# AdrianPerezHerrero/HDP-GPC

Hardware: AMD Instinct MI355X
Metric: GP log-lik evals/sec (NxK batch, T-point segments) (higher is better)
Workload: dtype f64; 1 GPU; BASELINE configs[1]: synthetic 2048 segments x 8 clusters, T=128, fp64, irregular segment grids (per-pair Gram + Cholesky + score); segments=2048, segments_per_gpu=2048, clusters=8, T=128

## Files before the change

### hdpgpc_amd/csrc/hgp_internal.hpp

```cpp
#pragma once
#include <hip/hip_runtime.h>
#include <stddef.h>
#include <stdint.h>
#include <stdlib.h>

#include <type_traits>
#include <vector>

#include "../../include/hdpgpc_hip.h"

constexpr int WAVES = 4;

static inline int launch_status() {
  hipError_t e = hipGetLastError();
  return e == hipSuccess ? 0 : 1000 + (int)e;
}

static inline int nb_for(int n) {
  int nb = (n + 15) / 16;
  nb = (nb + 1) & ~1;
  return nb < 2 ? 2 : nb;
}

template <class F> static inline auto dispatch_nb_wave(int T, F&& f) {
  switch (nb_for(T)) {
    case 2: return f(std::integral_constant<int, 2>{});
    case 4: return f(std::integral_constant<int, 4>{});
    case 6: return f(std::integral_constant<int, 6>{});
    default: return f(std::integral_constant<int, 8>{});
  }
}
template <class F> static inline auto dispatch_nb_coop(int T, F&& f) {
  return T <= 192 ? f(std::integral_constant<int, 12>{}) : f(std::integral_constant<int, 16>{});
}
template <class F> static inline auto dispatch_nb(int NB, F&& f) {
  return NB <= 8 ? dispatch_nb_wave(16 * NB, f) : dispatch_nb_coop(16 * NB, f);
}
template <class F> static inline auto dispatch_bool(bool on, F&& f) {
  return on ? f(std::true_type{}) : f(std::false_type{});
}

static inline bool env_on(const char* name) {
  const char* v = getenv(name);
  return v && v[0] && v[0] != '0';
}

constexpr double PAIRS_CUT = 55.45177444479562;
constexpr int PAIRS_FB_CAP = 65536;

static inline int acc_grid_for(int nb) { return nb > 8 ? 256 : 512; }

struct hgp_pairs_plan {
  int T, K, TP, NB;
  std::vector<double> theta;
  std::vector<int32_t> perm;
  std::vector<int> grp_beg, grp_end;
  std::vector<double> grp_ell;
  double *d_theta, *d_scal, *d_A, *d_S, *d_Z, *d_Kinv, *d_P, *d_Q, *d_Mp, *d_ap, *d_xb;
  int32_t* d_perm;
  bool coop = false;
  double* d_escr = nullptr;
  int32_t* d_eflags = nullptr;
  int nscr = 0;
  long escr_stride = 0;
  double acc_tol = 1e-9;
  double* d_Lop = nullptr;
  double* d_LTop = nullptr;
  double* d_Dop = nullptr;
  double* d_Sop = nullptr;
  double* d_mu = nullptr;
  int32_t* d_acc_list = nullptr;
  double* d_sscr = nullptr;
  int32_t* d_fb = nullptr;
  int score_out = 0;
};

struct PlanReuse {
  long long* key_jit;
  int32_t* valid;
  int32_t* same;
  int32_t* factored;
  int32_t* info;
  static constexpr size_t BYTES_PER_CLUSTER = sizeof(long long) + 4 * sizeof(int32_t);
};
static inline PlanReuse plan_reuse(const hgp_pairs_plan* p) {
  long long* key = reinterpret_cast<long long*>(p->d_Q);
  int32_t* w = reinterpret_cast<int32_t*>(key + p->K);
  return PlanReuse{key, w, w + p->K, w + 2 * p->K, w + 3 * p->K};
}

struct PotrfArgs {
  double* A;
  int T, b;
  double jitter_rel, add;
  double* Linv;
  double* logdet;
  int32_t* info;
  double* Aout = nullptr;
  const int32_t* src_idx = nullptr;
};
int hgp_internal_potrf_ws(const double* A, const int32_t* idx, int T, int b, double jitter_rel, double* L, int32_t* info, hipStream_t st);
int hgp_internal_potrf_coop(const PotrfArgs& a, hipStream_t st);

struct InvArgs {
  const double* A;
  int T, b;
  double jitter_rel, add;
  double* Linv;
  int32_t* info;
  const double* rhs = nullptr;
  int rhs_trans = 0;
  int symmetric = 0;
  const int32_t* rhs_on = nullptr;
  double* rhs_out = nullptr;
  const int32_t* keep = nullptr;
};
static_assert(offsetof(InvArgs, rhs_on) == 64, "InvArgs: the plain forms' arguments fill the first 64 bytes");
int hgp_internal_chol_inverse(const InvArgs& a, int NB, double* factor_out, hipStream_t st);
void hgp_internal_wave_inverse(const InvArgs& a, hipStream_t st);
void hgp_internal_trtri(const double* L, double* Z, int T, int b, const int32_t* info, hipStream_t st);
int hgp_internal_ensure_dynamic_lds(const void* fn, size_t bytes);

struct GemmArgs {
  const double* A;
  const double* B;
  double* C;
  int M, N, Kd, lda, ldb, ldc;
  long sA, sB, sC;
  double alpha, beta;
  int tA, tB;
  int nb2 = 1;
  long sA2 = 0, sB2 = 0, sC2 = 0;
  const double* D = nullptr;
  int ldd = 0;
  long sD = 0;
  int boff = 0;
  int triA = 0;
};
int hgp_internal_gemm(const GemmArgs& a, int batch, hipStream_t st);
void hgp_internal_dot_batched(const double* X, const double* Y, long sX, long sY, long n, double scale, int accumulate, double* out, int b, hipStream_t st);
void hgp_internal_colnorm_diag(const double* Z, const double* S, long sS, int T, double scale, int accumulate, double* out, int b, hipStream_t st);
void hgp_internal_sub_batched(const double* A, const double* B, long sA, long sB, long n, double* C, int b, hipStream_t st);

int hgp_internal_acc_prep(hgp_pairs_plan* p, const double* mean, bool flags_done, hipStream_t st);
int hgp_internal_pairs_acc(const hgp_pairs_plan* p, const double* x, const double* y, int N, int Ts, const double* first_noise,
                           const int32_t* sel, double* out_quad, double* out_logdet, int32_t* out_info, hipStream_t st);
int hgp_internal_pairs_acc_ragged(const hgp_pairs_plan* p, const double* x, const double* y, int N, int ld, const int32_t* seg_len,
                                  const double* first_noise, const int32_t* sel, double* out_quad, double* out_logdet,
                                  int32_t* out_info, hipStream_t st);
size_t hgp_internal_acc_bytes(int TP, int K, size_t* sizes );

int hgp_internal_lat_coop(const double* f_cur, const double* f_prev, const double* A, const double* Gamma, const double* P, int T, int b,
                          double* out, int32_t* info, double* ws, hipStream_t st);
int hgp_internal_mniw_coop(const double* M, const double* Sigma, const double* m_mean, const double* scale, long prior_stride, int T, int b,
                           double* out, int32_t* info, double* ws, hipStream_t st);

struct PairsArgs {
  const double* x;
  const double* y;
  int N, Ts;
  const double* xb;
  int T;
  const double* Mp;
  const double* ap;
  const double* scal;
  const int32_t* perm;
  int kbeg, kend;
  double ell;
  const double* first_noise;
  const int32_t* sel;
#ifdef HGP_STAMPS
  unsigned long long* stamps;
#endif
  int K;
  double* out_quad;
  double* out_logdet;
  int32_t* out_info;
  double* escr;
  int32_t* eflags;
  int nscr;
  long escr_stride;
  int flags;
  double score_add;
  int score_on;
  int32_t* fb;
};

struct PairsRagArgs : PairsArgs {
  const int32_t* seg_len;
};
template <class Args> constexpr bool pairs_ragged = std::is_base_of<PairsRagArgs, Args>::value;

struct PairsSegArgs : PairsArgs {
  const double* store;
};

#ifdef HGP_STAMPS
extern unsigned long long* hgp_internal_stamp_dev;
#endif
int hgp_internal_pairs_fast(const PairsArgs& a, int NB, bool coop, hipStream_t st);
int hgp_internal_pairs_fast_ragged(const PairsRagArgs& a, int NB, bool coop, hipStream_t st);
int hgp_internal_pairs_listed(const PairsArgs& a, int NB, hipStream_t st);
int hgp_internal_pairs_listed_ragged(const PairsRagArgs& a, int NB, hipStream_t st);
```

### hdpgpc_amd/csrc/hgp_pairs_acc.hip

```cpp
#include <hip/hip_runtime.h>
#include <math.h>
#include <stdint.h>

#include "hgp_internal.hpp"
#include "tile_f64.hpp"

using namespace hgp;

namespace {

__host__ __device__ constexpr int ntl(int NB) { return NB * (NB - 1) / 2; }
__host__ __device__ constexpr int tl(int K, int Kp) { return K * (K - 1) / 2 + Kp; }

#ifndef HGP_PAIRS_RAGGED_TU
__global__ void k_acc_flags(double* scal, int K, double tol, int32_t* acc_list) {
  if (threadIdx.x != 0 || blockIdx.x != 0) return;
  int n = 0;
  for (int k = 0; k < K; ++k) {
    const double ck = scal[8 * k] * scal[8 * k + 6];
    const double bound = F64_EPS * ck * ck;
    const bool flag = (tol == 0.0) || (tol > 0.0 && !(bound <= tol));
    scal[8 * k + 7] = flag ? 1.0 : 0.0;
    if (flag) acc_list[1 + n++] = k;
  }
  acc_list[0] = n;
}

template <int NB>
__global__ __launch_bounds__(64) void k_acc_factor(double* A, int TP, const double* scal, int32_t* info, int32_t* factored) {
  __shared__ __attribute__((aligned(16))) double scr[DIAG_SCR];
  const int k = blockIdx.x, lane = threadIdx.x;
  if (scal[8 * k + 7] == 0.0) return;
  if (factored[k] != 0) return;
  double* Ak = A + (size_t)k * TP * TP;
  d4 U[NB * (NB + 1) / 2];
  d4 R[NB];
  load_upper_only<NB>(U, Ak, TP, TP, lane);
  PivotAcc pa;
  pa.init();
  wave_factor<NB, 0>(U, R, scr, nullptr, nullptr, lane, pa, Ak, TP, TP);
  if (lane == 0 && info && pa.info != 0) info[k] = pa.info;
  if (lane == 0) factored[k] = 1;
}

struct AccPrepArgs {
  const double* L;
  const double* S;
  const double* mean;
  const double* scal;
  int T, TP, NB;
  double* Lop;
  double* LTop;
  double* Dop;
  double* Sop;
  double* mu;
};

__global__ __launch_bounds__(256) void k_acc_prep(AccPrepArgs a) {
  const int k = blockIdx.x;
  if (a.scal[8 * k + 7] == 0.0) return;
  const int lane = threadIdx.x & 63, g = lane >> 4, c = lane & 15;
  const int wv = blockIdx.y * 4 + (threadIdx.x >> 6), nwv = gridDim.y * 4;
  const int NB = a.NB, TP = a.TP;
  const double* L = a.L + (size_t)k * TP * TP;
  const double* S = a.S + (size_t)k * TP * TP;
  const int nl = ntl(NB);
  double* Lop = a.Lop + (size_t)k * nl * 256;
  double* LTop = a.LTop + (size_t)k * nl * 256;
  double* Dop = a.Dop + (size_t)k * 4 * NB * 256;
  double* Sop = a.Sop + (size_t)k * NB * NB * 256;
  if (blockIdx.y == 0)
    for (int i = threadIdx.x; i < TP; i += 256) a.mu[(size_t)k * TP + i] = (i < a.T) ? a.mean[(size_t)k * a.T + i] : 0.0;
  const int items = nl + NB + NB * NB;
  for (int it = wv; it < items; it += nwv) {
    if (it < nl) {
      int Kb = 1;
      while (tl(Kb + 1, 0) <= it) ++Kb;
      const int Kp = it - tl(Kb, 0);
      d4 lo, lt;
#pragma unroll
      for (int s = 0; s < 4; ++s) {
        lo[s] = L[(size_t)(16 * Kb + c) * TP + 16 * Kp + 4 * s + g];
        lt[s] = L[(size_t)(16 * Kb + 4 * s + g) * TP + 16 * Kp + c];
      }
      *reinterpret_cast<d4*>(Lop + ((size_t)it * 64 + lane) * 4) = lo;
      *reinterpret_cast<d4*>(LTop + ((size_t)it * 64 + lane) * 4) = lt;
    } else if (it < nl + NB) {
      const int Kb = it - nl;
      const double* D = L + (size_t)(16 * Kb) * TP + 16 * Kb;
      d4 a1, a2, a1t, a2t;
#pragma unroll
      for (int r = 0; r < 4; ++r) {
        const double* B = D + (size_t)(4 * r) * TP + 4 * r;
        const double l00 = B[0], l10 = B[TP], l11 = B[TP + 1], l20 = B[2 * TP], l21 = B[2 * TP + 1], l22 = B[2 * TP + 2],
                     l30 = B[3 * (size_t)TP], l31 = B[3 * (size_t)TP + 1], l32 = B[3 * (size_t)TP + 2], l33 = B[3 * (size_t)TP + 3];
        double w[4][4];
#pragma unroll
        for (int i = 0; i < 4; ++i)
#pragma unroll
          for (int j = 0; j < 4; ++j) w[i][j] = 0.0;
        const double r0 = 1.0 / l00, r1 = 1.0 / l11, r2 = 1.0 / l22, r3 = 1.0 / l33;
        w[0][0] = r0;
        w[1][0] = -(l10 * w[0][0]) * r1;
        w[2][0] = -(l20 * w[0][0] + l21 * w[1][0]) * r2;
        w[3][0] = -(l30 * w[0][0] + l31 * w[1][0] + l32 * w[2][0]) * r3;
        w[1][1] = r1;
        w[2][1] = -(l21 * w[1][1]) * r2;
        w[3][1] = -(l31 * w[1][1] + l32 * w[2][1]) * r3;
        w[2][2] = r2;
        w[3][2] = -(l32 * w[2][2]) * r3;
        w[3][3] = r3;
        const int ci = c & 3;
        double wf = 0.0, wt = 0.0;
#pragma unroll
        for (int i = 0; i < 4; ++i)
#pragma unroll
          for (int j = 0; j < 4; ++j) {
            if (i == ci && j == g) wf = w[i][j];
            if (i == g && j == ci) wt = w[i][j];
          }
        const bool mine = (c >> 2) == r;
        a1[r] = mine ? wf : 0.0;
        a1t[r] = mine ? wt : 0.0;
        a2[r] = (c >= 4 * r + 4) ? D[(size_t)c * TP + 4 * r + g] : 0.0;
        a2t[r] = (c < 4 * r) ? D[(size_t)(4 * r + g) * TP + c] : 0.0;
      }
      *reinterpret_cast<d4*>(Dop + ((size_t)(0 * NB + Kb) * 64 + lane) * 4) = a1;
      *reinterpret_cast<d4*>(Dop + ((size_t)(1 * NB + Kb) * 64 + lane) * 4) = a2;
      *reinterpret_cast<d4*>(Dop + ((size_t)(2 * NB + Kb) * 64 + lane) * 4) = a1t;
      *reinterpret_cast<d4*>(Dop + ((size_t)(3 * NB + Kb) * 64 + lane) * 4) = a2t;
    } else {
      const int t = it - nl - NB, Kb = t / NB, Kp = t % NB;
      d4 so;
#pragma unroll
      for (int s = 0; s < 4; ++s) so[s] = S[(size_t)(16 * Kp + 4 * s + g) * TP + 16 * Kb + c];
      *reinterpret_cast<d4*>(Sop + ((size_t)t * 64 + lane) * 4) = so;
    }
  }
}

#endif

struct AccArgs {
  const double* x;
  const double* y;
  int N, Ts;
  const double* xb;
  int T;
  const double* scal;
  const double* mu;
  const double* Lop;
  const double* LTop;
  const double* Dop;
  const double* Sop;
  const int32_t* acc_list;
  const double* first_noise;
  const int32_t* sel;
  int K;
  double* out_quad;
  double* out_logdet;
  int32_t* out_info;
  double* sscr;
  double score_add;
  int score_on;
};
struct AccRagArgs : AccArgs {
  const int32_t* seg_len;
};
template <class Args> constexpr bool acc_ragged = std::is_base_of<AccRagArgs, Args>::value;
#ifdef HGP_PAIRS_RAGGED_TU
using KArgs = AccRagArgs;
#define ACC_SEG_LEN(a, n, ld) __builtin_amdgcn_readfirstlane((a).seg_len[n])
#define ACC_SCORE_ADD(a, Ts) (-0.5 * (double)(Ts) * 1.8378770664093453)
#else
using KArgs = AccArgs;
#define ACC_SEG_LEN(a, n, ld) (ld)
#define ACC_SCORE_ADD(a, Ts) (a).score_add
#endif

template <int NB>
struct PairsAccLds {
  static constexpr int TP = 16 * NB;
  static constexpr int ROWBUF = 0, WBUF = ROWBUF + NB * 256, DVEC = WBUF + 256, XS = DVEC + TP, YS = XS + TP, XBS = YS + TP,
                       MUS = XBS + TP, SCR = MUS + TP, RED = SCR + DIAG_SCR, REDI = RED + 32;
  static constexpr size_t BYTES = sizeof(double) * REDI + sizeof(int) * 16;
  static_assert(WBUF % 2 == 0 && SCR % 2 == 0 && BYTES <= LDS_MAX_BYTES, "k_pairs_acc: LDS");
  HGP_LDS_DOUBLES(rowbuf, ROWBUF)
  HGP_LDS_DOUBLES(Wbuf, WBUF)
  HGP_LDS_DOUBLES(dvec, DVEC)
  HGP_LDS_DOUBLES(xs, XS)
  HGP_LDS_DOUBLES(ys, YS)
  HGP_LDS_DOUBLES(xbs, XBS)
  HGP_LDS_DOUBLES(mus, MUS)
  HGP_LDS_DOUBLES(scr, SCR)
  HGP_LDS_DOUBLES(red, RED)
  HGP_LDS_INTS(redi, REDI, 0)
};

__device__ __forceinline__ d4 ld4(const double* base, unsigned off) { return *reinterpret_cast<const d4*>(base + off); }

template <int NB>
__global__ __launch_bounds__(64 * CoopH<NB>::NW, (NB <= 8) ? 2 : 1) void k_pairs_acc(KArgs a) {
  using H = CoopH<NB>;
  constexpr int NW = H::NW, TP = 16 * NB;
  extern __shared__ __attribute__((aligned(16))) double smem[];
  using L = PairsAccLds<NB>;
  double *rowbuf = L::rowbuf(smem), *Wbuf = L::Wbuf(smem), *dvec = L::dvec(smem), *xs = L::xs(smem), *ys = L::ys(smem);
  double *xbs = L::xbs(smem), *mus = L::mus(smem), *scr = L::scr(smem), *red = L::red(smem);
  int* redi = L::redi(smem);
  const int tid = threadIdx.x, lane = tid & 63, g = lane >> 4, c = lane & 15;
  const int wave = __builtin_amdgcn_readfirstlane(tid >> 6);
  const int T = a.T, row_ld = a.Ts;
  const int nflag = a.acc_list[0];
  if (nflag == 0) return;
  const long npairs = a.sel ? (long)a.N : (long)a.N * nflag;
  double* Ssc = a.sscr + (size_t)blockIdx.x * NB * NB * 256;

  for (long p = blockIdx.x; p < npairs; p += gridDim.x) {
    int n, kc;
    if (a.sel) {
      n = (int)p;
      kc = a.sel[n];
      if (a.scal[8 * kc + 7] == 0.0) continue;
    } else {
      n = (int)(p / nflag);
      kc = a.acc_list[1 + (int)(p % nflag)];
    }
    kc = __builtin_amdgcn_readfirstlane(kc);
    const double* sc = a.scal + 8 * kc;
    const double cc = sc[0], ell = sc[1], noise = sc[2];
    const bool iso = sc[3] != 0.0;
    const size_t oidx = a.sel ? (size_t)n : (size_t)n * a.K + kc;
    const double fn = a.first_noise ? a.first_noise[oidx] : 0.0;
    const int Ts = ACC_SEG_LEN(a, n, row_ld);
    if constexpr (acc_ragged<KArgs>) {
      if (Ts < 1 || Ts > row_ld) {
        if (tid == 0) {
          a.out_quad[oidx] = __builtin_nan("");
          if (a.out_logdet) a.out_logdet[oidx] = __builtin_nan("");
          if (a.out_info) a.out_info[oidx] = -1;
        }
        continue;
      }
    }
    __syncthreads();
    for (int i = tid; i < TP; i += 64 * NW) {
      xs[i] = (i < Ts) ? a.x[(size_t)n * row_ld + i] / ell : 1e150 * (double)(1 + i);
      ys[i] = (i < Ts) ? a.y[(size_t)n * row_ld + i] : 0.0;
      xbs[i] = (i < T) ? a.xb[i] / ell : -1e150 * (double)(1 + i);
      mus[i] = a.mu[(size_t)kc * TP + i];
    }
    __syncthreads();
    const double* Lop = a.Lop + (size_t)kc * ntl(NB) * 256;
    const double* LTop = a.LTop + (size_t)kc * ntl(NB) * 256;
    const double* Dop = a.Dop + (size_t)kc * 4 * NB * 256;
    const double* Sop = a.Sop + (size_t)kc * NB * NB * 256;
    double* Sl = Ssc;

    double dsq = 0.0;
#pragma unroll
    for (int q = 0; q < 2; ++q) {
      const int J = (q == 0) ? wave : NB - 1 - wave;
      d4 X[NB];
#pragma unroll
      for (int K = 0; K < NB; ++K) {
        const unsigned l4 = (unsigned)launder(lane) * 4u;
        {
          const int ln = launder(lane);
          const double xj = xs[16 * J + (ln & 15)];
#pragma unroll
          for (int r = 0; r < 4; ++r) {
            const double u = xbs[16 * K + 4 * r + (ln >> 4)] - xj;
            X[K][r] = cc * exp(-0.5 * (u * u));
          }
        }
#pragma unroll
        for (int Kp = 0; Kp < K; ++Kp) {
          const d4 lo = ld4(Lop + tl(K, Kp) * 256, l4);
#pragma unroll
          for (int s = 0; s < 4; ++s) X[K] = mfma_sub(lo[s], X[Kp][s], X[K]);
        }
        const d4 a1 = ld4(Dop + (0 * NB + K) * 256, l4), a2 = ld4(Dop + (1 * NB + K) * 256, l4);
#pragma unroll
        for (int r = 0; r < 4; ++r) {
          d4 t = X[K];
          t[r] = 0.0;
          t = mfma(a1[r], X[K][r], t);
          X[K] = (r < 3) ? mfma_sub(a2[r], t[r], t) : t;
        }
      }
#pragma unroll
      for (int K = NB - 1; K >= 0; --K) {
        const unsigned l4 = (unsigned)launder(lane) * 4u;
#pragma unroll
        for (int Kp = NB - 1; Kp > K; --Kp) {
          const d4 lt = ld4(LTop + tl(Kp, K) * 256, l4);
#pragma unroll
          for (int s = 0; s < 4; ++s) X[K] = mfma_sub(lt[s], X[Kp][s], X[K]);
        }
        const d4 a1 = ld4(Dop + (2 * NB + K) * 256, l4), a2 = ld4(Dop + (3 * NB + K) * 256, l4);
#pragma unroll
        for (int r = 3; r >= 0; --r) {
          d4 t = X[K];
          t[r] = 0.0;
          t = mfma(a1[r], X[K][r], t);
          X[K] = (r > 0) ? mfma_sub(a2[r], t[r], t) : t;
        }
      }
      double pj = 0.0;
#pragma unroll
      for (int K = 0; K < NB; ++K) {
        const int ln = launder(lane);
        const unsigned l4 = (unsigned)ln * 4u;
#pragma unroll
        for (int r = 0; r < 4; ++r) pj = fma(X[K][r], mus[16 * K + 4 * r + (ln >> 4)], pj);
        *reinterpret_cast<d4*>(Sl + (K * NB + J) * 256 + l4) = X[K];
      }
      pj = xrow_sum(pj);
      if (g == 0) {
        const int j = 16 * J + c;
        const double d = ys[j] - pj;
        dvec[j] = d;
        dsq = fma(d, d, dsq);
      }
    }
    __syncthreads();

    if (iso) {
      dsq = wave_sum(dsq);
      if (lane == 0) red[wave] = dsq;
      __syncthreads();
      if (tid == 0) {
        const double v = sc[4] + fn;
        const double v2 = v + 1e-8 * fmax(fabs(v), F64_EPS);
        double tot_ = 0.0;
        for (int w_ = 0; w_ < NW; ++w_) tot_ += red[w_];
        a.out_quad[oidx] = a.score_on ? fma(-0.5, tot_ / v2, ACC_SCORE_ADD(a, Ts)) : (tot_ / v2);
        if (a.out_logdet) a.out_logdet[oidx] = (double)Ts * log(v2);
        if (a.out_info) a.out_info[oidx] = (v2 > 0.0) ? 0 : 1;
      }
      continue;
    }

    d4 U[H::NT];
#pragma unroll
    for (int q = 0; q < 2; ++q) {
      const int J = (q == 0) ? wave : NB - 1 - wave;
      const double xj = xs[16 * J + c];
#pragma unroll
      for (int I = 0; I < (q == 0 ? NW : NB); ++I) {
        const int ln = launder(lane);
        d4 kt = (d4){0.0, 0.0, 0.0, 0.0};
        if (I <= J) {
#pragma unroll
          for (int r = 0; r < 4; ++r) {
            const double u = xs[16 * I + (ln >> 4) + 4 * r] - xs[16 * J + (ln & 15)];
            kt[r] = cc * exp(-0.5 * (u * u));
          }
          if (I == J) {
#pragma unroll
            for (int r = 0; r < 4; ++r)
              if ((ln >> 4) + 4 * r == (ln & 15)) kt[r] = (16 * I + (ln & 15) < Ts) ? cc + noise : 1.0;
          }
          U[q == 0 ? H::slotA(I) : H::slotB(I)] = kt;
        }
      }
#pragma nounroll
      for (int K = 0; K < NB; ++K) {
        const unsigned l4 = (unsigned)launder(lane) * 4u;
        d4 Q;
#pragma unroll
        for (int r = 0; r < 4; ++r) {
          const double u = xbs[16 * K + 4 * r + g] - xj;
          Q[r] = -(cc * exp(-0.5 * (u * u)));
        }
#pragma unroll
        for (int Kp = 0; Kp < NB; ++Kp) {
          const d4 so = ld4(Sop + (K * NB + Kp) * 256, l4);
          const d4 sb = ld4(Sl + (Kp * NB + J) * 256, l4);
#pragma unroll
          for (int s = 0; s < 4; ++s) Q = mfma(so[s], sb[s], Q);
        }
#pragma unroll
        for (int I = 0; I < (q == 0 ? NW : NB); ++I) {
          if (I <= J) {
            const d4 sa = ld4(Sl + (K * NB + I) * 256, l4);
#pragma unroll
            for (int s = 0; s < 4; ++s)
              U[q == 0 ? H::slotA(I) : H::slotB(I)] = mfma(sa[s], Q[s], U[q == 0 ? H::slotA(I) : H::slotB(I)]);
          }
        }
      }
    }

    cooph_regularise<NB>(U, 1e-6 + fn, 1e-8, Ts, wave, lane, red);
    PivotAcc pa;
    pa.init();
    double zq = cooph_factor<NB>(U, rowbuf, Wbuf, scr, wave, lane, pa, Ts, dvec);
    int info;
    const double ld = cooph_logdet_info<NB>(pa, wave, lane, red, redi, info);
    zq = wave_sum(zq);
    if (lane == 0) red[8 + wave] = zq;
    __syncthreads();
    if (tid == 0) {
      double tot_ = 0.0;
      for (int w_ = 0; w_ < NW; ++w_) tot_ += red[8 + w_];
      a.out_quad[oidx] = a.score_on ? fma(-0.5, tot_, ACC_SCORE_ADD(a, Ts)) : (tot_);
      if (a.out_logdet) a.out_logdet[oidx] = ld;
      if (a.out_info) a.out_info[oidx] = info;
    }
  }
}

template <int NB>
int launch_pairs_acc(const KArgs& a, hipStream_t st) {
  const size_t lds = PairsAccLds<NB>::BYTES;
  hipLaunchKernelGGL(k_pairs_acc<NB>, dim3(acc_grid_for(NB)), dim3(64 * CoopH<NB>::NW), lds, st, a);
  return launch_status();
}

AccArgs acc_args(const hgp_pairs_plan* p, const double* x, const double* y, int N, int Ts, const double* first_noise, const int32_t* sel,
                 double* out_quad, double* out_logdet, int32_t* out_info) {
  return AccArgs{x, y, N, Ts, p->d_xb, p->T, p->d_scal, p->d_mu, p->d_Lop, p->d_LTop, p->d_Dop, p->d_Sop, p->d_acc_list,
                 first_noise, sel, p->K, out_quad, out_logdet, out_info, p->d_sscr, -0.5 * (double)Ts * 1.8378770664093453, p->score_out};
}

}

#ifdef HGP_PAIRS_RAGGED_TU
int hgp_internal_pairs_acc_ragged(const hgp_pairs_plan* p, const double* x, const double* y, int N, int ld, const int32_t* seg_len,
                                  const double* first_noise, const int32_t* sel, double* out_quad, double* out_logdet,
                                  int32_t* out_info, hipStream_t st) {
  if (p->acc_tol < 0.0) return 0;
  const AccRagArgs a{acc_args(p, x, y, N, ld, first_noise, sel, out_quad, out_logdet, out_info), seg_len};
  return dispatch_nb(p->NB, [&](auto nb) { return launch_pairs_acc<decltype(nb)::value>(a, st); });
}
#else
size_t hgp_internal_acc_bytes(int TP, int K, size_t* sizes) {
  const int NB = TP / 16;
  size_t s[6];
  s[0] = (size_t)K * ntl(NB) * 256 * sizeof(double);
  s[1] = s[0];
  s[2] = (size_t)K * 4 * NB * 256 * sizeof(double);
  s[3] = (size_t)K * NB * NB * 256 * sizeof(double);
  s[4] = (size_t)K * TP * sizeof(double);
  s[5] = (size_t)acc_grid_for(NB) * NB * NB * 256 * sizeof(double);
  size_t tot = 0;
  for (int i = 0; i < 6; ++i) {
    if (sizes) sizes[i] = s[i];
    tot += (s[i] + 255) & ~(size_t)255;
  }
  return tot;
}

int hgp_internal_acc_prep(hgp_pairs_plan* p, const double* mean, bool flags_done, hipStream_t st) {
  const int K = p->K, TP = p->TP, NB = p->NB;
  if (!flags_done) hipLaunchKernelGGL(k_acc_flags, dim3(1), dim3(64), 0, st, p->d_scal, K, p->acc_tol, p->d_acc_list);
  if (p->acc_tol < 0.0) return launch_status();
  if (NB <= 8)
    dispatch_nb_wave(TP, [&](auto nb) {
      hipLaunchKernelGGL(k_acc_factor<decltype(nb)::value>, dim3(K), dim3(64), 0, st, p->d_A, TP, p->d_scal, (int32_t*)nullptr,
                         plan_reuse(p).factored);
    });
  AccPrepArgs a{p->d_A, p->d_S, mean, p->d_scal, p->T, TP, NB, p->d_Lop, p->d_LTop, p->d_Dop, p->d_Sop, p->d_mu};
  hipLaunchKernelGGL(k_acc_prep, dim3(K, 8), dim3(256), 0, st, a);
  return launch_status();
}

int hgp_internal_pairs_acc(const hgp_pairs_plan* p, const double* x, const double* y, int N, int Ts, const double* first_noise,
                           const int32_t* sel, double* out_quad, double* out_logdet, int32_t* out_info, hipStream_t st) {
  if (p->acc_tol < 0.0) return 0;
  const AccArgs a = acc_args(p, x, y, N, Ts, first_noise, sel, out_quad, out_logdet, out_info);
  return dispatch_nb(p->NB, [&](auto nb) { return launch_pairs_acc<decltype(nb)::value>(a, st); });
}
#endif
```

### hdpgpc_amd/csrc/hgp_plan.hip

```cpp
#include <algorithm>
#include <new>

#include "../../include/hdpgpc_hip_ragged.h"
#include "hgp_internal.hpp"
#include "tile_f64.hpp"

using namespace hgp;

namespace {

struct PrepArgs {
  const double* xb;
  const double* mean;
  const double* Sigma;
  int T, TP, K;
  const double* theta;
  double* scal;
  double* A;
  double* S;
  double* xb_copy;
  PlanReuse reuse;
  int32_t* info;
};

__global__ __launch_bounds__(256) void k_prep_build(PrepArgs a) {
  __shared__ double red[256];
  __shared__ int redi[256];
  const int k = blockIdx.x, tid = threadIdx.x;
  const int T = a.T, TP = a.TP;
  const double* Sg = a.Sigma + (size_t)k * T * T;
  const double c = a.theta[3 * k], ell = a.theta[3 * k + 1], noise = a.theta[3 * k + 2];
  double s_abs = 0.0, s_sgn = 0.0;
  for (int i = tid; i < T; i += 256) {
    double d = Sg[(size_t)i * T + i];
    s_abs += fabs(d);
    s_sgn += d;
  }
  red[tid] = s_abs;
  __syncthreads();
  for (int o = 128; o > 0; o >>= 1) {
    if (tid < o) red[tid] += red[tid + o];
    __syncthreads();
  }
  const double mean_abs = red[0] / T;
  __syncthreads();
  red[tid] = s_sgn;
  __syncthreads();
  for (int o = 128; o > 0; o >>= 1) {
    if (tid < o) red[tid] += red[tid + o];
    __syncthreads();
  }
  const double mS = red[0] / T;
  int bad = 0;
  for (int i = tid; i < T; i += 256) {
    double d = Sg[(size_t)i * T + i];
    if (!(fabs(d - mS) <= 1e-8 + 1e-5 * fabs(mS))) bad = 1;
  }
  const bool reuse = a.reuse.same != nullptr;
  if (reuse) {
    const long long* xn = reinterpret_cast<const long long*>(a.xb);
    const long long* xo = reinterpret_cast<const long long*>(a.xb_copy);
    for (int i = tid; i < T; i += 256)
      if (xn[i] != xo[i]) bad |= 2;
  }
  redi[tid] = bad;
  __syncthreads();
  for (int o = 128; o > 0; o >>= 1) {
    if (tid < o) redi[tid] |= redi[tid + o];
    __syncthreads();
  }
  const double jit = 1e-4 * fmax(mean_abs, F64_EPS);
  const bool same = reuse && (redi[0] & 2) == 0 && a.reuse.valid[k] != 0 && a.reuse.key_jit[k] == __double_as_longlong(jit);
  if (tid == 0 && blockIdx.y == 0) {
    double* sc = a.scal + 8 * k;
    sc[0] = c;
    sc[1] = ell;
    sc[2] = noise;
    sc[3] = (redi[0] & 1) ? 0.0 : 1.0;
    sc[4] = mS;
    sc[5] = jit;
    sc[6] = 0.0;
    if (reuse) {
      a.reuse.same[k] = same ? 1 : 0;
      if (same) {
        if (a.info) a.info[k] = a.reuse.info[k];
      } else {
        a.reuse.valid[k] = 0;
        a.reuse.factored[k] = 0;
      }
    }
  }
  if (!reuse && k == 0 && blockIdx.y == 0)
    for (int i = tid; i < TP; i += 256) a.xb_copy[i] = (i < T) ? a.xb[i] : 0.0;
  double* Ak = a.A + (size_t)k * TP * TP;
  double* Sk = a.S + (size_t)k * TP * TP;
  if (same) {
    for (int idx = blockIdx.y * 256 + tid; idx < TP * TP; idx += gridDim.y * 256) {
      int i = idx / TP, j = idx % TP;
      double sv = 0.0;
      if (i < T && j < T) sv = 0.5 * (Sg[(size_t)i * T + j] + Sg[(size_t)j * T + i]);
      Sk[idx] = sv;
    }
    return;
  }
  for (int idx = blockIdx.y * 256 + tid; idx < TP * TP; idx += gridDim.y * 256) {
    int i = idx / TP, j = idx % TP;
    double av, sv = 0.0;
    if (i < T && j < T) {
      double u = a.xb[i] / ell - a.xb[j] / ell;
      av = c * exp(-0.5 * (u * u));
      if (i == j) av += jit;
      sv = 0.5 * (Sg[(size_t)i * T + j] + Sg[(size_t)j * T + i]);
    } else {
      av = (i == j) ? 1.0 : 0.0;
    }
    Ak[idx] = av;
    Sk[idx] = sv;
  }
}

__device__ __forceinline__ double plan_mp_value(double c, double qij, double qji, double kij, double kji) {
  return (c * c) * (0.5 * (qij + qji) - 0.5 * (kij + kji));
}
__device__ __forceinline__ int plan_mp_col(int j, int NHh) {
  const int hh = j / (16 * NHh), tl = (j / 16) % NHh, cc = j % 16;
  const int loc = (tl < 2 * (NHh / 2)) ? 32 * (tl / 2) + 2 * cc + (tl & 1) : 16 * (NHh - 1) + cc;
  return 16 * NHh * hh + loc;
}

struct PrepFinalArgs {
  const double* Q;
  const double* Kinv;
  const double* mean;
  double* scal;
  int T, TP;
  double* Mp;
  double* ap;
  int interleave;
  int32_t* fb;
};

__global__ __launch_bounds__(256) void k_prep_final(PrepFinalArgs a) {
  const int k = blockIdx.x, tid = threadIdx.x;
  if (a.fb && k == 0 && blockIdx.y == 0 && tid == 0) {
    a.fb[0] = 0;
    a.fb[1 + PAIRS_FB_CAP] = 0;
  }
  const int T = a.T, TP = a.TP;
  const double c = a.scal[8 * k];
  const double* Q = a.Q + (size_t)k * TP * TP;
  const double* Ki = a.Kinv + (size_t)k * TP * TP;
  double* Mp = a.Mp + (size_t)k * TP * TP;
  __shared__ double tq[32][33], tk[32][33];
  const int NHh = (TP / 16) / 2, nt = TP / 32;
  const int tx = tid & 31, ty = tid >> 5;
  for (int t = blockIdx.y; t < nt * nt; t += gridDim.y) {
    const int bi = t / nt, bj = t % nt;
    __syncthreads();
#pragma unroll
    for (int r = 0; r < 4; ++r) {
      const int y = ty + 8 * r;
      tq[y][tx] = Q[(size_t)(32 * bj + y) * TP + 32 * bi + tx];
      tk[y][tx] = Ki[(size_t)(32 * bj + y) * TP + 32 * bi + tx];
    }
    __syncthreads();
#pragma unroll
    for (int r = 0; r < 4; ++r) {
      const int y = ty + 8 * r;
      const int i = 32 * bi + y, j = 32 * bj + tx;
      double v = 0.0;
      if (i < T && j < T) v = plan_mp_value(c, Q[(size_t)i * TP + j], tq[tx][y], Ki[(size_t)i * TP + j], tk[tx][y]);
      const int jp = a.interleave ? plan_mp_col(j, NHh) : j;
      Mp[(size_t)i * TP + jp] = v;
    }
  }
  const double* mu = a.mean + (size_t)k * T;
  __shared__ double red[256];
  double rmax = 0.0;
  for (int i = blockIdx.y * 256 + tid; i < TP; i += gridDim.y * 256) {
    double s = 0.0, rs = 0.0;
    if (i < T) {
#pragma unroll 8
      for (int j = 0; j < T; ++j) {
        const double kij = Ki[(size_t)j * TP + i];
        s = fma(kij, mu[j], s);
        rs += fabs(kij);
      }
    }
    a.ap[(size_t)k * TP + i] = c * s;
    rmax = fmax(rmax, rs);
  }
  red[tid] = rmax;
  __syncthreads();
  for (int o = 128; o > 0; o >>= 1) {
    if (tid < o) red[tid] = fmax(red[tid], red[tid + o]);
    __syncthreads();
  }
  if (tid == 0) atomicMax(reinterpret_cast<unsigned long long*>(a.scal + 8 * k + 6), (unsigned long long)__double_as_longlong(red[0]));
}

struct PlanOpsArgs {
  const double* Z;
  const double* S;
  const double* mean;
  double* scal;
  int T, K;
  double* Mp;
  double* ap;
  double tol;
  int32_t* acc_list;
  int32_t* fb;
  unsigned* done;
  double* Kinv;
  PlanReuse reuse;
  const double* xb;
  double* xb_copy;
  const int32_t* info;
};

template <int NB>
struct PlanOpsLds {
  static constexpr int TILE = 256;
  static constexpr int TILE_T = 16 * 17;
  static constexpr int COL = 0, ROW = COL + 2 * NB * TILE, P = ROW + 2 * NB * TILE_T, END = P + 2 * NB * TILE;
  static constexpr int QT = END, DOUBLES = END + 4 * TILE_T;
  static constexpr size_t BYTES = (size_t)DOUBLES * sizeof(double);
};

__device__ inline void plan_acc_flags(double* scal, int K, double tol, int32_t* acc_list) {
  int n = 0;
  for (int k = 0; k < K; ++k) {
    const double ninf = __longlong_as_double((long long)__hip_atomic_load(
        reinterpret_cast<unsigned long long*>(scal + 8 * k + 6), __ATOMIC_RELAXED, __HIP_MEMORY_SCOPE_AGENT));
    const double ck = scal[8 * k] * ninf;
    const double bound = F64_EPS * ck * ck;
    const bool flag = (tol == 0.0) || (tol > 0.0 && !(bound <= tol));
    scal[8 * k + 7] = flag ? 1.0 : 0.0;
    if (flag) acc_list[1 + n++] = k;
  }
  acc_list[0] = n;
}

template <int NB>
__global__ __launch_bounds__(128 * NB) void k_plan_ops(PlanOpsArgs a) {
  using L = PlanOpsLds<NB>;
  constexpr int TP = 16 * NB, NK = 4 * NB, NOFF = NB * (NB - 1) / 2;
  constexpr int TRIP = (NB == 6) ? 12 : (NB == 2 ? 8 : 16);
  extern __shared__ __attribute__((aligned(16))) double smem[];
  __shared__ int last;
  const int tid = threadIdx.x, lane = tid & 63, g = lane >> 4, c = lane & 15;
  const int wave = __builtin_amdgcn_readfirstlane(tid >> 6);
  const int k = blockIdx.x / NOFF;
  int I, J = 1;
  {
    int t = blockIdx.x % NOFF;
    while (t >= J) t -= J++;
    I = t;
  }
  const bool dI = J == I + 1, dJ = dI && J == NB - 1;
  const int T = a.T;
  const double* Z = a.Z + (size_t)k * TP * TP;
  const double* S = a.S + (size_t)k * TP * TP;
  double* colS = smem + L::COL;
  double* rowS = smem + L::ROW;
  double* pS = smem + L::P;
  double* qT = smem + L::QT;
  const int q = wave / NB, wa = wave % NB;
  const int Bq = q ? J : I;

  const bool same = a.reuse.same[k] != 0;
  {
    double* Kc = a.Kinv + (size_t)k * TP * TP + (wa * NB + Bq) * L::TILE + lane * 4;
    d4 ccol = (d4){0.0, 0.0, 0.0, 0.0}, crow = (d4){0.0, 0.0, 0.0, 0.0};
    if (same) {
      ccol = *reinterpret_cast<const d4*>(Kc);
      crow = *reinterpret_cast<const d4*>(a.Kinv + (size_t)k * TP * TP + (Bq * NB + wa) * L::TILE + lane * 4);
    } else {
      const double* Za = Z + 16 * wa + c;
      const double* Zb = Z + 16 * Bq + c;
#pragma unroll
      for (int k0 = 0; k0 < NK; k0 += TRIP) {
        double za[TRIP], zb[TRIP];
#pragma unroll
        for (int u = 0; u < TRIP; ++u) {
          const int kk = 4 * (k0 + u) + g;
          za[u] = Za[(size_t)kk * TP];
          zb[u] = Zb[(size_t)kk * TP];
        }
        __builtin_amdgcn_sched_barrier(0);
#pragma unroll
        for (int u = 0; u < TRIP; ++u) {
          ccol = mfma(za[u], zb[u], ccol);
          crow = mfma(zb[u], za[u], crow);
        }
      }
      if (q == 0 ? dI : dJ) *reinterpret_cast<d4*>(Kc) = ccol;
    }
    *reinterpret_cast<d4*>(colS + (q * NB + wa) * L::TILE + lane * 4) = ccol;
#pragma unroll
    for (int r = 0; r < 4; ++r) rowS[(q * NB + wa) * L::TILE_T + (g + 4 * r) * 17 + c] = crow[r];
  }
  __syncthreads();

  {
    const double* Scol = S + (size_t)g * TP + 16 * wa + c;
    const double* cs = colS + q * NB * L::TILE + lane * 4;
    d4 acc = (d4){0.0, 0.0, 0.0, 0.0};
#pragma unroll
    for (int k0 = 0; k0 < NK; k0 += TRIP) {
      double sv[TRIP];
#pragma unroll
      for (int u = 0; u < TRIP; ++u) sv[u] = Scol[(size_t)(4 * (k0 + u)) * TP];
      __builtin_amdgcn_sched_barrier(0);
#pragma unroll
      for (int u = 0; u < TRIP; ++u) acc = mfma(sv[u], cs[((k0 + u) >> 2) * L::TILE + ((k0 + u) & 3)], acc);
    }
    *reinterpret_cast<d4*>(pS + (q * NB + wa) * L::TILE + lane * 4) = acc;
  }
  __syncthreads();

  if (wave < 2 || (wave == 2 && dI) || (wave == 3 && dJ)) {
    const int sr = wave & 1, sp = (wave < 2) ? 1 - sr : sr;
    const double* rs_ = rowS + sr * NB * L::TILE_T + c * 17 + g;
    const double* ps = pS + sp * NB * L::TILE + lane * 4;
    d4 acc = (d4){0.0, 0.0, 0.0, 0.0};
#pragma unroll
    for (int u = 0; u < NK; ++u) acc = mfma(rs_[(u >> 2) * L::TILE_T + 4 * (u & 3)], ps[(u >> 2) * L::TILE + (u & 3)], acc);
#pragma unroll
    for (int r = 0; r < 4; ++r) qT[wave * L::TILE_T + (g + 4 * r) * 17 + c] = acc[r];
  }
  constexpr int WA = NB > 2 ? 4 : 2;
  if ((wave == WA && dI) || (wave == WA + 1 && dJ)) {
    const int sq = wave - WA;
    const double* cs = colS + sq * NB * L::TILE;
    const double cc = a.scal[8 * k];
    const double* mu = a.mean + (size_t)k * T;
    const int i = 16 * (sq ? J : I) + c;
    double s = 0.0, rs = 0.0;
    if (g == 0 && i < T) {
#pragma unroll 8
      for (int j = 0; j < T; ++j) {
        const int jj = j & 15;
        const double kij = cs[(j >> 4) * L::TILE + (16 * (jj & 3) + c) * 4 + (jj >> 2)];
        s = fma(kij, mu[j], s);
        rs += fabs(kij);
      }
    }
    if (g == 0) a.ap[(size_t)k * TP + i] = cc * s;
    const double rmax = wave_allreduce<true>(fmax(0.0, rs));
    if (lane == 0) atomicMax(reinterpret_cast<unsigned long long*>(a.scal + 8 * k + 6), (unsigned long long)__double_as_longlong(rmax));
  }
  __syncthreads();

  {
    const double cc = a.scal[8 * k];
    double* Mp = a.Mp + (size_t)k * TP * TP;
    constexpr int NHh = NB / 2;
    for (int e = tid; e < 1024; e += 128 * NB) {
      const int m = e >> 8, rr = (e >> 4) & 15, c2 = e & 15;
      if ((m == 2 && !dI) || (m == 3 && !dJ)) continue;
      const int sm = m & 1, so = (m < 2) ? 1 - sm : sm;
      const int bi = sm ? J : I, bj = so ? J : I;
      const int qa = m, qb = (m < 2) ? 1 - m : m;
      const int i = 16 * bi + rr, j = 16 * bj + c2;
      double v = 0.0;
      if (i < T && j < T)
        v = plan_mp_value(cc, qT[qa * L::TILE_T + rr * 17 + c2], qT[qb * L::TILE_T + c2 * 17 + rr],
                          rowS[(sm * NB + bj) * L::TILE_T + rr * 17 + c2], rowS[(so * NB + bi) * L::TILE_T + c2 * 17 + rr]);
      Mp[(size_t)i * TP + plan_mp_col(j, NHh)] = v;
    }
  }

  if (!dI) return;
  if (!same && I == 0) {
    if (tid == 0) {
      a.reuse.key_jit[k] = __double_as_longlong(a.scal[8 * k + 5]);
      a.reuse.info[k] = a.info ? a.info[k] : 0;
    }
    if (k == 0)
      for (int i = tid; i < TP; i += 128 * NB) a.xb_copy[i] = (i < T) ? a.xb[i] : 0.0;
  }
  __syncthreads();
  if (tid == 0) {
    __threadfence();
    last = atomicAdd(a.done, 1u) == (unsigned)(a.K * (NB - 1)) - 1u ? 1 : 0;
  }
  __syncthreads();
  if (last && tid == 0) {
    __threadfence();
    plan_acc_flags(a.scal, a.K, a.tol, a.acc_list);
    a.fb[0] = 0;
    a.fb[1 + PAIRS_FB_CAP] = 0;
    *a.done = 0u;
    for (int kk = 0; kk < a.K; ++kk) a.reuse.valid[kk] = 1;
  }
}

template <int NB>
int launch_plan_ops(const PlanOpsArgs& a, hipStream_t st) {
  const size_t lds = PlanOpsLds<NB>::BYTES;
  if (int rc = hgp_internal_ensure_dynamic_lds(reinterpret_cast<const void*>(&k_plan_ops<NB>), lds)) return rc;
  hipLaunchKernelGGL(k_plan_ops<NB>, dim3(a.K * (NB * (NB - 1) / 2)), dim3(128 * NB), lds, st, a);
  return launch_status();
}

static int tp_for(int n) {
  if (n <= HGP_MAX_T_WAVE) return 16 * nb_for(n);
  return n <= 192 ? 192 : 256;
}

size_t plan_layout(hgp_pairs_plan* p, int T, int Ts_max, int K, char* base) {
  const size_t TP = (size_t)tp_for(std::max(T, Ts_max));
  const size_t mat = (size_t)K * TP * TP * sizeof(double);
  p->TP = (int)TP;
  p->NB = p->TP / 16;
  p->coop = p->TP > HGP_MAX_T_WAVE;
  size_t o = 0;
  auto take = [&](auto*& member, size_t bytes) {
    if (base) member = reinterpret_cast<std::remove_reference_t<decltype(member)>>(base + o);
    o += (bytes + 255) & ~(size_t)255;
  };
  take(p->d_theta, (size_t)K * 3 * sizeof(double));
  take(p->d_scal, (size_t)K * 8 * sizeof(double));
  take(p->d_A, mat);
  take(p->d_S, mat);
  take(p->d_Z, mat);
  take(p->d_Kinv, mat);
  take(p->d_P, mat);
  take(p->d_Q, mat);
  take(p->d_Mp, mat);
  take(p->d_ap, (size_t)K * TP * sizeof(double));
  take(p->d_perm, (size_t)K * sizeof(int32_t));
  take(p->d_xb, TP * sizeof(double));
  if (p->coop) {
    const size_t nb = (size_t)p->NB;
    const size_t cap = (nb >= 12) ? 48 : (nb == 8 ? 24 : 16);
    const size_t over = nb * nb > cap ? nb * nb - cap : 0;
    p->nscr = over ? (nb >= 12 ? 512 : 1024) : 0;
    p->escr_stride = (long)(over * 256);
    take(p->d_escr, (size_t)p->nscr * over * 256 * sizeof(double));
    take(p->d_eflags, ((size_t)p->nscr + 1) * sizeof(int32_t));
  }
  size_t sz[6];
  hgp_internal_acc_bytes((int)TP, K, sz);
  take(p->d_Lop, sz[0]);
  take(p->d_LTop, sz[1]);
  take(p->d_Dop, sz[2]);
  take(p->d_Sop, sz[3]);
  take(p->d_mu, sz[4]);
  take(p->d_sscr, sz[5]);
  take(p->d_acc_list, (size_t)(K + 1) * sizeof(int32_t));
  take(p->d_fb, (size_t)(PAIRS_FB_CAP + 2) * sizeof(int32_t));
  return o;
}

}

#ifdef HGP_STAMPS
unsigned long long* hgp_internal_stamp_dev = nullptr;
#endif

extern "C" {

size_t hgp_pairs_plan_device_bytes(int T, int Ts_max, int K) {
  if (T <= 0 || Ts_max <= 0 || K <= 0) return 0;
  hgp_pairs_plan sizing;
  return plan_layout(&sizing, T, Ts_max, K, nullptr);
}

int hgp_pairs_plan_create(hgp_pairs_plan** plan, int T, int Ts_max, int K, const double* theta_host, void* dev_buf,
                          size_t dev_bytes) {
  if (!plan || !theta_host || !dev_buf || T <= 0 || Ts_max <= 0 || K <= 0) return -1;
  if (T > HGP_MAX_T_COOP || Ts_max > HGP_MAX_T_COOP) return -2;
  if (dev_bytes < hgp_pairs_plan_device_bytes(T, Ts_max, K)) return -1;
  for (int k = 0; k < K; ++k)
    if (!(theta_host[3 * k] > 0.0) || !(theta_host[3 * k + 1] > 0.0)) return -1;
  hgp_pairs_plan* p = new (std::nothrow) hgp_pairs_plan();
  if (!p) return -1;
  p->T = T;
  p->K = K;
  p->theta.assign(theta_host, theta_host + 3 * (size_t)K);
  p->perm.resize(K);
  for (int k = 0; k < K; ++k) p->perm[k] = k;
  std::stable_sort(p->perm.begin(), p->perm.end(),
                   [&](int a, int b) { return p->theta[3 * a + 1] < p->theta[3 * b + 1]; });
  for (int i = 0; i < K;) {
    int j = i;
    double ell = p->theta[3 * p->perm[i] + 1];
    while (j < K && p->theta[3 * p->perm[j] + 1] == ell) ++j;
    p->grp_beg.push_back(i);
    p->grp_end.push_back(j);
    p->grp_ell.push_back(ell);
    i = j;
  }
  plan_layout(p, T, Ts_max, K, (char*)dev_buf);
  if (hipMemset(p->d_fb, 0, (size_t)(PAIRS_FB_CAP + 2) * sizeof(int32_t)) != hipSuccess) {
    delete p;
    return 1000 + (int)hipGetLastError();
  }
  if (!p->coop && hipMemset(p->d_P, 0, 256) != hipSuccess) {
    delete p;
    return 1000 + (int)hipGetLastError();
  }
  if (!p->coop && hipMemset(p->d_Q, 0, (size_t)K * PlanReuse::BYTES_PER_CLUSTER) != hipSuccess) {
    delete p;
    return 1000 + (int)hipGetLastError();
  }
  if (p->coop && hipMemset(p->d_eflags, 0, (p->nscr + 1) * sizeof(int32_t)) != hipSuccess) {
    delete p;
    return 1000 + (int)hipGetLastError();
  }
  if (hipMemcpy(p->d_theta, p->theta.data(), sizeof(double) * 3 * K, hipMemcpyHostToDevice) != hipSuccess ||
      hipMemcpy(p->d_perm, p->perm.data(), sizeof(int32_t) * K, hipMemcpyHostToDevice) != hipSuccess) {
    delete p;
    return 1000 + (int)hipGetLastError();
  }
  *plan = p;
  return 0;
}

void hgp_pairs_plan_destroy(hgp_pairs_plan* plan) { delete plan; }

const double* hgp_pairs_plan_scalars(const hgp_pairs_plan* plan) { return plan ? plan->d_scal : nullptr; }

int hgp_pairs_plan_update(hgp_pairs_plan* p, const double* x_basis, const double* mean, const double* Sigma,
                          int32_t* info, void* stream) {
  if (!p || !x_basis || !mean || !Sigma) return -1;
  hipStream_t st = (hipStream_t)stream;
  const int K = p->K, T = p->T, TP = p->TP;
  const PlanReuse reuse = p->coop ? PlanReuse{} : plan_reuse(p);
  PrepArgs pa{x_basis, mean, Sigma, T, TP, K, p->d_theta, p->d_scal, p->d_A, p->d_S, p->d_xb, reuse, info};
  hipLaunchKernelGGL(k_prep_build, dim3(K, 8), dim3(256), 0, st, pa);
  InvArgs fa{p->d_A, TP, K, 0.0, 0.0, p->d_Z, info};
  fa.symmetric = 1;
  fa.keep = reuse.same;
  if (int rc = hgp_internal_chol_inverse(fa, p->NB, p->d_A, st)) return rc;
  if (!p->coop) {
    PlanOpsArgs oa{p->d_Z, p->d_S, mean, p->d_scal, T, K, p->d_Mp, p->d_ap, p->acc_tol, p->d_acc_list, p->d_fb,
                   reinterpret_cast<unsigned*>(p->d_P), p->d_Kinv, reuse, x_basis, p->d_xb, info};
    if (int rc = dispatch_nb_wave(TP, [&](auto nb) { return launch_plan_ops<decltype(nb)::value>(oa, st); })) return rc;
    int rc = hgp_internal_acc_prep(p, mean, true, st);
    return rc ? rc : launch_status();
  }
  const long sm = (long)TP * TP;
  GemmArgs g1{p->d_Z, p->d_Z, p->d_Kinv, TP, TP, TP, TP, TP, TP, sm, sm, sm, 1.0, 0.0, 1, 0};
  GemmArgs g2{p->d_S, p->d_Kinv, p->d_P, TP, TP, TP, TP, TP, TP, sm, sm, sm, 1.0, 0.0, 0, 0};
  GemmArgs g3{p->d_Kinv, p->d_P, p->d_Q, TP, TP, TP, TP, TP, TP, sm, sm, sm, 1.0, 0.0, 0, 0};
  hgp_internal_gemm(g1, K, st);
  hgp_internal_gemm(g2, K, st);
  hgp_internal_gemm(g3, K, st);
  PrepFinalArgs fin{p->d_Q, p->d_Kinv, mean, p->d_scal, T, TP, p->d_Mp, p->d_ap, p->coop ? 0 : 1, p->d_fb};
  hipLaunchKernelGGL(k_prep_final, dim3(K, 8), dim3(256), 0, st, fin);
  if (p->d_eflags && p->nscr > 0 && hipMemsetAsync(p->d_eflags, 0, (p->nscr + 1) * sizeof(int32_t), st) != hipSuccess) return launch_status();
  int rc = hgp_internal_acc_prep(p, mean, false, st);
  return rc ? rc : launch_status();
}

int hgp_pairs_plan_set_accuracy(hgp_pairs_plan* p, double tol) {
  if (!p || tol != tol) return -1;
  p->acc_tol = tol;
  return 0;
}

int hgp_pairs_plan_set_score_output(hgp_pairs_plan* p, int on) {
  if (!p) return -1;
  p->score_out = on ? 1 : 0;
  return 0;
}

static int loglik_pairs(const hgp_pairs_plan* p, const double* x, const double* y, int N, int ld, const int32_t* seg_len,
                        const double* first_noise, const int32_t* sel, double* out_quad, double* out_logdet, int32_t* out_info,
                        void* stream) {
  const int Ts = ld;
  if (Ts > HGP_MAX_T_COOP) return -2;
  if (Ts > p->TP) return -2;
  hipStream_t st = (hipStream_t)stream;
  int rc = 0;
  if (p->coop && p->d_eflags && p->nscr > 0 &&
      hipMemsetAsync(p->d_eflags, 0, (p->nscr + 1) * sizeof(int32_t), st) != hipSuccess)
    return launch_status();
  for (size_t gi = 0; gi < p->grp_beg.size() && rc == 0; ++gi) {
    PairsArgs a{x, y, N, Ts, p->d_xb, p->T, p->d_Mp, p->d_ap, p->d_scal, p->d_perm, p->grp_beg[gi], p->grp_end[gi],
                p->grp_ell[gi], first_noise, sel,
#ifdef HGP_STAMPS
                hgp_internal_stamp_dev,
#endif
                p->K, out_quad, out_logdet, out_info, p->d_escr, p->d_eflags, p->nscr, p->escr_stride,
                env_on("HGP_PAIRS_GENERIC") ? 1 : 0, -0.5 * (double)Ts * 1.8378770664093453, p->score_out, p->d_fb};
    rc = seg_len ? hgp_internal_pairs_fast_ragged(PairsRagArgs{a, seg_len}, p->NB, p->coop, st)
                 : hgp_internal_pairs_fast(a, p->NB, p->coop, st);
  }
  if (rc == 0)
    rc = seg_len ? hgp_internal_pairs_acc_ragged(p, x, y, N, ld, seg_len, first_noise, sel, out_quad, out_logdet, out_info, st)
                 : hgp_internal_pairs_acc(p, x, y, N, Ts, first_noise, sel, out_quad, out_logdet, out_info, st);
  return rc;
}

int hgp_loglik_pairs_f64(const hgp_pairs_plan* p, const double* x, const double* y, int N, int Ts,
                         const double* first_noise, const int32_t* sel, double* out_quad, double* out_logdet,
                         int32_t* out_info, void* stream) {
  if (N == 0) return 0;
  if (!p || !x || !y || !out_quad || N < 0 || Ts <= 0) return -1;
  return loglik_pairs(p, x, y, N, Ts, nullptr, first_noise, sel, out_quad, out_logdet, out_info, stream);
}

int hgp_loglik_pairs_ragged_f64(const hgp_pairs_plan* p, const double* x, const double* y, int N, int ld, const int32_t* seg_len,
                                const double* first_noise, const int32_t* sel, double* out_quad, double* out_logdet,
                                int32_t* out_info, void* stream) {
  if (N == 0) return 0;
  if (!p || !x || !y || !seg_len || !out_quad || N < 0 || ld <= 0) return -1;
  return loglik_pairs(p, x, y, N, ld, seg_len, first_noise, sel, out_quad, out_logdet, out_info, stream);
}

#ifdef HGP_STAMPS
int hgp_debug_stamps(unsigned long long* out8_host) {
  if (!hgp_internal_stamp_dev) {
    if (hipMalloc(&hgp_internal_stamp_dev, 128) != hipSuccess) return 1;
    (void)hipMemset(hgp_internal_stamp_dev, 0, 128);
  }
  if (hipMemcpy(out8_host, hgp_internal_stamp_dev, 128, hipMemcpyDeviceToHost) != hipSuccess) return 1;
  (void)hipMemset(hgp_internal_stamp_dev, 0, 128);
  return 0;
}
#endif

}
```

Measured before the change: 18.42 million evals/s.

## Skip plan-ops and acc-prep recomputation when cluster state is unchanged across calls

Adds per-cluster change detection: the plan-build kernel compares the freshly symmetrised S and the mean against stored copies and flags clusters whose state differs. Plan-ops blocks for unchanged clusters exit early, restoring the cached ninf value and bumping the completion counter by the full pair count. Acc-prep blocks also skip work via per-block packed flags. This avoids repeated Gram-derived operator construction across evaluations, at the cost of extra compare traffic and more complex cross-kernel state bookkeeping. That bookkeeping risks staleness bugs.

```diff
diff --git a/hdpgpc_amd/csrc/hgp_internal.hpp b/hdpgpc_amd/csrc/hgp_internal.hpp
--- a/hdpgpc_amd/csrc/hgp_internal.hpp
+++ b/hdpgpc_amd/csrc/hgp_internal.hpp
@@ -81,12 +81,22 @@
   int32_t* same;
   int32_t* factored;
   int32_t* info;
-  static constexpr size_t BYTES_PER_CLUSTER = sizeof(long long) + 4 * sizeof(int32_t);
+  double* ninf;
+  int32_t* differs;
+  int32_t* state_valid;
+  int32_t* packed;
+  int32_t* state_same;
+  double* mean_copy;
+  static constexpr int ACC_PREP_GY = 8;
+  static constexpr size_t BYTES_PER_CLUSTER = 2 * sizeof(long long) + (7 + ACC_PREP_GY) * sizeof(int32_t);
 };
 static inline PlanReuse plan_reuse(const hgp_pairs_plan* p) {
+  const int K = p->K;
   long long* key = reinterpret_cast<long long*>(p->d_Q);
-  int32_t* w = reinterpret_cast<int32_t*>(key + p->K);
-  return PlanReuse{key, w, w + p->K, w + 2 * p->K, w + 3 * p->K};
+  int32_t* w = reinterpret_cast<int32_t*>(key + K);
+  double* ninf = reinterpret_cast<double*>(w + 4 * K);
+  int32_t* v = reinterpret_cast<int32_t*>(ninf + K);
+  return PlanReuse{key, w, w + K, w + 2 * K, w + 3 * K, ninf, v, v + K, v + 2 * K, v + (2 + PlanReuse::ACC_PREP_GY) * K, p->d_P + 32};
 }
 
 struct PotrfArgs {
diff --git a/hdpgpc_amd/csrc/hgp_pairs_acc.hip b/hdpgpc_amd/csrc/hgp_pairs_acc.hip
--- a/hdpgpc_amd/csrc/hgp_pairs_acc.hip
+++ b/hdpgpc_amd/csrc/hgp_pairs_acc.hip
@@ -54,11 +54,14 @@
   double* Dop;
   double* Sop;
   double* mu;
+  int32_t* packed;
 };
 
+template <bool KEEP>
 __global__ __launch_bounds__(256) void k_acc_prep(AccPrepArgs a) {
   const int k = blockIdx.x;
   if (a.scal[8 * k + 7] == 0.0) return;
+  if (KEEP && a.packed[gridDim.y * k + blockIdx.y] != 0) return;
   const int lane = threadIdx.x & 63, g = lane >> 4, c = lane & 15;
   const int wv = blockIdx.y * 4 + (threadIdx.x >> 6), nwv = gridDim.y * 4;
   const int NB = a.NB, TP = a.TP;
@@ -135,6 +138,13 @@
 #pragma unroll
       for (int s = 0; s < 4; ++s) so[s] = S[(size_t)(16 * Kp + 4 * s + g) * TP + 16 * Kb + c];
       *reinterpret_cast<d4*>(Sop + ((size_t)t * 64 + lane) * 4) = so;
+    }
+  }
+  if (KEEP) {
+    __syncthreads();
+    if (threadIdx.x == 0) {
+      __threadfence();
+      a.packed[gridDim.y * k + blockIdx.y] = 1;
     }
   }
 }
@@ -462,8 +472,12 @@
       hipLaunchKernelGGL(k_acc_factor<decltype(nb)::value>, dim3(K), dim3(64), 0, st, p->d_A, TP, p->d_scal, (int32_t*)nullptr,
                          plan_reuse(p).factored);
     });
-  AccPrepArgs a{p->d_A, p->d_S, mean, p->d_scal, p->T, TP, NB, p->d_Lop, p->d_LTop, p->d_Dop, p->d_Sop, p->d_mu};
-  hipLaunchKernelGGL(k_acc_prep, dim3(K, 8), dim3(256), 0, st, a);
+  AccPrepArgs a{p->d_A, p->d_S, mean, p->d_scal, p->T, TP, NB, p->d_Lop, p->d_LTop, p->d_Dop, p->d_Sop, p->d_mu,
+                NB <= 8 ? plan_reuse(p).packed : nullptr};
+  if (NB <= 8)
+    hipLaunchKernelGGL(k_acc_prep<true>, dim3(K, PlanReuse::ACC_PREP_GY), dim3(256), 0, st, a);
+  else
+    hipLaunchKernelGGL(k_acc_prep<false>, dim3(K, 8), dim3(256), 0, st, a);
   return launch_status();
 }
 
diff --git a/hdpgpc_amd/csrc/hgp_plan.hip b/hdpgpc_amd/csrc/hgp_plan.hip
--- a/hdpgpc_amd/csrc/hgp_plan.hip
+++ b/hdpgpc_amd/csrc/hgp_plan.hip
@@ -94,14 +94,51 @@
     for (int i = tid; i < TP; i += 256) a.xb_copy[i] = (i < T) ? a.xb[i] : 0.0;
   double* Ak = a.A + (size_t)k * TP * TP;
   double* Sk = a.S + (size_t)k * TP * TP;
-  if (same) {
-    for (int idx = blockIdx.y * 256 + tid; idx < TP * TP; idx += gridDim.y * 256) {
-      int i = idx / TP, j = idx % TP;
-      double sv = 0.0;
-      if (i < T && j < T) sv = 0.5 * (Sg[(size_t)i * T + j] + Sg[(size_t)j * T + i]);
-      Sk[idx] = sv;
-    }
-    return;
+  if (reuse) {
+    int diff = same ? 0 : 1;
+    const long long* mn = reinterpret_cast<const long long*>(a.mean + (size_t)k * T);
+    long long* mo = reinterpret_cast<long long*>(a.reuse.mean_copy + (size_t)k * T);
+    constexpr int NV = 8;
+    double sv[NV];
+    if (same) {
+      const long long* So = reinterpret_cast<const long long*>(Sk);
+      long long so[NV];
+#pragma unroll
+      for (int u = 0; u < NV; ++u) {
+        const int idx = (u * (int)gridDim.y + (int)blockIdx.y) * 256 + tid;
+        sv[u] = 0.0;
+        so[u] = 0;
+        if (idx < TP * TP) {
+          const int i = idx / TP, j = idx % TP;
+          if (i < T && j < T) sv[u] = 0.5 * (Sg[(size_t)i * T + j] + Sg[(size_t)j * T + i]);
+          so[u] = So[idx];
+        }
+      }
+#pragma unroll
+      for (int u = 0; u < NV; ++u)
+        if (__double_as_longlong(sv[u]) != so[u]) diff = 1;
+      if (blockIdx.y == 0)
+        for (int i = tid; i < T; i += 256)
+          if (mn[i] != mo[i]) diff = 1;
+    }
+    if (!__syncthreads_or(diff)) return;
+    if (tid == 0) {
+      atomicOr(a.reuse.differs + k, 1);
+      a.reuse.state_valid[k] = 0;
+    }
+    if (tid < PlanReuse::ACC_PREP_GY) a.reuse.packed[PlanReuse::ACC_PREP_GY * k + tid] = 0;
+    __threadfence();
+    __syncthreads();
+    if (blockIdx.y == 0)
+      for (int i = tid; i < T; i += 256) mo[i] = mn[i];
+    if (same) {
+#pragma unroll
+      for (int u = 0; u < NV; ++u) {
+        const int idx = (u * (int)gridDim.y + (int)blockIdx.y) * 256 + tid;
+        if (idx < TP * TP) Sk[idx] = sv[u];
+      }
+      return;
+    }
   }
   for (int idx = blockIdx.y * 256 + tid; idx < TP * TP; idx += gridDim.y * 256) {
     int i = idx / TP, j = idx % TP;
@@ -242,21 +279,12 @@
 }
 
 template <int NB>
-__global__ __launch_bounds__(128 * NB) void k_plan_ops(PlanOpsArgs a) {
+__device__ __forceinline__ void plan_ops_pair(const PlanOpsArgs& a, double* smem, int k, int I, int J, bool same) {
   using L = PlanOpsLds<NB>;
-  constexpr int TP = 16 * NB, NK = 4 * NB, NOFF = NB * (NB - 1) / 2;
+  constexpr int TP = 16 * NB, NK = 4 * NB;
   constexpr int TRIP = (NB == 6) ? 12 : (NB == 2 ? 8 : 16);
-  extern __shared__ __attribute__((aligned(16))) double smem[];
-  __shared__ int last;
   const int tid = threadIdx.x, lane = tid & 63, g = lane >> 4, c = lane & 15;
   const int wave = __builtin_amdgcn_readfirstlane(tid >> 6);
-  const int k = blockIdx.x / NOFF;
-  int I, J = 1;
-  {
-    int t = blockIdx.x % NOFF;
-    while (t >= J) t -= J++;
-    I = t;
-  }
   const bool dI = J == I + 1, dJ = dI && J == NB - 1;
   const int T = a.T;
   const double* Z = a.Z + (size_t)k * TP * TP;
@@ -268,7 +296,6 @@
   const int q = wave / NB, wa = wave % NB;
   const int Bq = q ? J : I;
 
-  const bool same = a.reuse.same[k] != 0;
   {
     double* Kc = a.Kinv + (size_t)k * TP * TP + (wa * NB + Bq) * L::TILE + lane * 4;
     d4 ccol = (d4){0.0, 0.0, 0.0, 0.0}, crow = (d4){0.0, 0.0, 0.0, 0.0};
@@ -371,8 +398,7 @@
     }
   }
 
-  if (!dI) return;
-  if (!same && I == 0) {
+  if (!same && dI && I == 0) {
     if (tid == 0) {
       a.reuse.key_jit[k] = __double_as_longlong(a.scal[8 * k + 5]);
       a.reuse.info[k] = a.info ? a.info[k] : 0;
@@ -380,10 +406,38 @@
     if (k == 0)
       for (int i = tid; i < TP; i += 128 * NB) a.xb_copy[i] = (i < T) ? a.xb[i] : 0.0;
   }
+}
+
+template <int NB>
+__global__ __launch_bounds__(128 * NB) void k_plan_ops(PlanOpsArgs a) {
+  constexpr int NOFF = NB * (NB - 1) / 2;
+  extern __shared__ __attribute__((aligned(16))) double smem[];
+  __shared__ int last;
+  const int tid = threadIdx.x;
+  const int k = blockIdx.x / NOFF;
+  int I, J = 1;
+  {
+    int t = blockIdx.x % NOFF;
+    while (t >= J) t -= J++;
+    I = t;
+  }
+  const bool same = a.reuse.same[k] != 0;
+  const bool kept = same && a.reuse.differs[k] == 0 && a.reuse.state_valid[k] != 0;
+  const bool first = I == 0 && J == 1, dI = J == I + 1;
+  if (kept && !first) return;
+  if (first && tid == 0) a.reuse.state_same[k] = kept ? 1 : 0;
+  if (!kept) {
+    plan_ops_pair<NB>(a, smem, k, I, J, same);
+    if (!dI) asm volatile("s_waitcnt vmcnt(0)" ::: "memory");
+  } else if (tid == 0) {
+    atomicMax(reinterpret_cast<unsigned long long*>(a.scal + 8 * k + 6), (unsigned long long)__double_as_longlong(a.reuse.ninf[k]));
+  }
+
   __syncthreads();
   if (tid == 0) {
-    __threadfence();
-    last = atomicAdd(a.done, 1u) == (unsigned)(a.K * (NB - 1)) - 1u ? 1 : 0;
+    if (kept || dI) __threadfence();
+    const unsigned inc = kept ? (unsigned)NOFF : 1u;
+    last = atomicAdd(a.done, inc) + inc == (unsigned)(a.K * NOFF) ? 1 : 0;
   }
   __syncthreads();
   if (last && tid == 0) {
@@ -392,7 +446,14 @@
     a.fb[0] = 0;
     a.fb[1 + PAIRS_FB_CAP] = 0;
     *a.done = 0u;
-    for (int kk = 0; kk < a.K; ++kk) a.reuse.valid[kk] = 1;
+    for (int kk = 0; kk < a.K; ++kk) {
+      a.reuse.ninf[kk] = __longlong_as_double((long long)__hip_atomic_load(
+          reinterpret_cast<unsigned long long*>(a.scal + 8 * kk + 6), __ATOMIC_RELAXED, __HIP_MEMORY_SCOPE_AGENT));
+      a.reuse.differs[kk] = 0;
+      a.reuse.valid[kk] = 1;
+    }
+    __threadfence();
+    for (int kk = 0; kk < a.K; ++kk) a.reuse.state_valid[kk] = 1;
   }
 }
 
```

Result: faster. 18.70 million evals/s, median of 6 (+1.5%).
